# brian-kelley/CUDA-QR

Measured on AMD Instinct MI355X. Metric: fp64 GFLOP/s (% of roofline) + ||A-QR||_F/||A||_F, m x n QR at 1/2/4/8 GPUs, higher is better.
Workload: dtype f64; 1 GPU; C3: 16384x16384 square fp64 QR on 1 MI355X, nb=256; m=16384, n=16384, m_per_gpu=16384, nb=256, ib=32, input_buffers=31, input=uniform[0,1) counter-hash generator, seed 12+i, resident in HBM, collective=none

## Files before the change

### cuda-qr_amd/__init__.py

```python
import ctypes as C
import os

import numpy as np

HERE = os.path.dirname(os.path.abspath(__file__))
_which = os.environ.get("CUDA_QR_AMD_LIB", "")
LAB = _which == "lab" or _which.endswith(".so")
LAB_LIB_PATH = os.path.join(HERE, "libmi355xqr_lab.so")
LIB_PATH = (os.path.join(HERE, _which) if _which.endswith(".so") else LAB_LIB_PATH) if LAB else os.path.join(HERE, "libmi355xqr.so")
HEADER = os.path.join(os.path.dirname(HERE), "include", "mi355x_qr.h")

if not os.path.exists(LIB_PATH):
    raise ImportError(
        f"{LIB_PATH} is missing: build it with `make -C {HERE} all lab` (or python -c 'import __graft_entry__ as g; "
        "g.build()').  The HIP extension is mandatory; there is no CPU fallback.")

try:
    import torch
except Exception:
    pass

lib = C.CDLL(LIB_PATH)

QR_PROF_CLASSES = 4
# ... 39 lines not shown
_sig("qr_strerror", C.c_char_p, C.c_int)
_sig("qr_set_block_size", C.c_int, C.c_int, C.c_int)
_sig("qr_get_block_size", None, C.POINTER(C.c_int), C.POINTER(C.c_int))
_sig("qr_default_block_size", C.c_int, C.c_int, C.c_int, C.POINTER(C.c_int), C.POINTER(C.c_int))
_sig("qr_thin", C.c_int, _dp, C.c_int, C.c_int, _dp, _dp, C.c_int, C.c_int)
_fp = C.POINTER(C.c_float)
_sig("mmqr_f32_status", C.c_int, _fp, C.POINTER(_fp), C.c_int, C.c_int)
_sig("explicitQR_f32_status", C.c_int, _fp, _fp, _fp, _fp, C.c_int, C.c_int)
_sig("qr_thin_mgpu", C.c_int, _dp, C.c_int, C.c_int, _dp, _dp, C.c_int, C.c_int)
_sig("qr_release_cached_plans", C.c_int)
_sig("qr_tsqr_unique_id", C.c_int, _vp)
_sig("qr_tsqr_plan_create", C.c_int, C.POINTER(_vp), _vp, C.c_int, C.c_int, C.c_int, C.c_int, C.c_int)
_sig("qr_tsqr_plan_create_comm", C.c_int, C.POINTER(_vp), _vp, C.c_int, C.c_int, C.c_int, C.c_int, C.c_int)
_sig("qr_tsqr_plan_destroy", C.c_int, _vp)
_sig("qr_tsqr_factor_dev", C.c_int, _vp, _vp, C.c_int, _vp)
_sig("qr_tsqr_formq_dev", C.c_int, _vp, _vp, C.c_int, _vp, C.c_int)
_sig("qr_tsqr_local_dev", C.c_int, _vp, _vp, C.c_int)
_sig("qr_tsqr_exchange_buffers", C.c_int, _vp, C.POINTER(_vp), C.POINTER(_vp))
_sig("qr_tsqr_stacked_dev", C.c_int, _vp, _vp)
_sig("qr_tsqr_is_pipelined", C.c_int, _vp)
_sig("qr_tsqr_set_schedule", C.c_int, _vp, C.c_int)
_sig("qr_tsqr_gather_stats", C.c_int, _vp, C.POINTER(C.c_double))
_sig("qr_tsqr_factor_virtual_dev", C.c_int, C.POINTER(_vp), C.c_int, C.POINTER(_vp), C.c_int, C.POINTER(_vp))
_sig("qr_tsqr_factor_selfgather_dev", C.c_int, _vp, _vp, C.c_int, _vp)
_sig("qr_tsqr_sync", C.c_int, _vp)
_sig("qr_tsqr_stream", _vp, _vp)
_sig("qr_tsqr_comm_ranks", C.c_int, _vp, C.POINTER(C.c_int))
_sig("qr_tsqr_local_plan", _vp, _vp)
_sig("qr_tsqr_stacked_plan", _vp, _vp)
_sig("qr_plan_create", C.c_int, C.POINTER(_vp), C.c_int, C.c_int, C.c_int, C.c_int)
_sig("qr_plan_destroy", C.c_int, _vp)
_sig("qr_geqrf_dev", C.c_int, _vp, _vp, C.c_int, C.c_int, C.c_int, _vp)
_sig("qr_applyq_dev", C.c_int, _vp, _vp, C.c_int, C.c_int, C.c_int, _vp, _vp, C.c_int, C.c_int, C.c_int)
_sig("qr_build_t_dev", C.c_int, _vp, _vp, C.c_int, C.c_int, C.c_int, _vp, _vp, C.c_int)
_sig("qr_ormqr_dev", C.c_int, _vp, C.c_char, _vp, C.c_int, C.c_int, C.c_int, _vp, _vp, C.c_int, _vp, C.c_int, C.c_int)
_sig("qr_solve_r_dev", C.c_int, _vp, _vp, C.c_int, C.c_int, _vp, C.c_int, C.c_int)
_sig("qr_gels_dev", C.c_int, _vp, _vp, C.c_int, C.c_int, C.c_int, _vp, _vp, C.c_int, C.c_int)
_sig("qr_lstsq", C.c_int, _dp, C.c_int, C.c_int, _dp, C.c_int, _dp, _dp)
_sig("qr_extract_r_dev", C.c_int, _vp, _vp, C.c_int, C.c_int, C.c_int, _vp, C.c_int, C.c_int)
_sig("qr_gemm_dev", C.c_int, _vp, C.c_char, C.c_int, C.c_int, C.c_int, C.c_double, _vp, C.c_int, _vp, C.c_int,
     C.c_double, _vp, C.c_int)
_sig("qr_fill_uniform_dev", C.c_int, _vp, _vp, C.c_int, C.c_longlong, C.c_int, C.c_longlong, C.c_longlong,
     C.c_ulonglong)
_sig("qr_uniform_at", C.c_double, C.c_ulonglong, C.c_ulonglong)
_sig("qr_diffnorm_dev", C.c_int, _vp, _vp, C.c_int, _vp, C.c_int, C.c_longlong, C.c_int, C.c_longlong,
     C.c_longlong, C.c_ulonglong, C.c_int, _dp)
_sig("qr_device_malloc", C.c_int, C.POINTER(_vp), C.c_size_t)
_sig("qr_device_free", C.c_int, _vp)
_sig("qr_copy_to_device", C.c_int, _vp, _vp, C.c_size_t)
_sig("qr_copy_to_host", C.c_int, _vp, _vp, C.c_size_t)
_sig("qr_plan_sync", C.c_int, _vp)
_sig("qr_plan_stream", _vp, _vp)
_sig("qr_plan_set_guard_mode", C.c_int, _vp, C.c_int)
_sig("qr_plan_route_stats", C.c_int, _vp, C.POINTER(C.c_longlong))
_sig("qr_plan_retry_stats", C.c_int, _vp, C.POINTER(C.c_longlong))
_sig("qr_plan_info", C.c_int, _vp, C.POINTER(C.c_int), C.POINTER(C.c_int), C.POINTER(C.c_int))
_sig("qr_plan_update_cus", C.c_int, _vp)
_sig("qr_plan_set_profile", C.c_int, _vp, C.c_int)
_sig("qr_plan_pause_profile", C.c_int, _vp, C.c_int)
_sig("qr_plan_get_profile", C.c_int, _vp, C.POINTER(Profile))
_sig("qr_plan_get_profile_records", C.c_int, _vp, C.c_int, C.POINTER(C.c_int), _dp, _dp)
_sig("qr_device_info", C.c_int, C.c_char_p, C.c_int, C.POINTER(C.c_int), C.POINTER(C.c_int), C.POINTER(C.c_size_t))
_sig("qr_probe_mfma_f64_tflops", C.c_int, _dp)
_sig("qr_probe_copy_gbps", C.c_int, _dp)
_sig("qrd_gemm_nn", C.c_int, _vp, C.c_int, C.c_int, C.c_int, C.c_double, _vp, C.c_int, _vp, C.c_int, C.c_double,
     _vp, C.c_int)
_sig("qrd_gemm_tn", C.c_int, _vp, C.c_int, C.c_int, C.c_int, C.c_double, _vp, C.c_int, _vp, C.c_int, C.c_double,
     _vp, C.c_int, _vp, C.c_size_t, _vp, C.c_int)
_sig("qrd_gemm_tn_update", C.c_int, _vp, C.c_int, C.c_int, C.c_int, C.c_double, _vp, C.c_int, _vp, C.c_int, C.c_double,
     _vp, C.c_int, _vp, C.c_size_t)
_sig("qrd_gemm_tn_update_wide", C.c_int, _vp, C.c_int, C.c_int, C.c_int, C.c_double, _vp, C.c_int, _vp, C.c_int, C.c_double,
     _vp, C.c_int, _vp, C.c_size_t)
_sig("qrd_gemm_tn_dual", C.c_int, _vp, C.c_int, C.c_int, C.c_int, _vp, C.c_int, _vp, C.c_int, _vp, C.c_int, _vp, C.c_int, _vp, C.c_int, _vp, C.c_int,
     _vp, C.c_size_t)
_sig("qrd_trsm_gt", C.c_int, _vp, C.c_int, C.c_int, _vp, C.c_int, _vp, C.c_int, _vp, C.c_int, _vp, C.c_int)
_sig("qrd_larft", C.c_int, _vp, C.c_int, C.c_int, _vp, C.c_int, _vp, _vp, C.c_int, _vp, C.c_int, _vp, C.c_int)
_sig("qrd_panel_ws_size", C.c_size_t, C.c_int)
_sig("qrd_panel_tsqr", C.c_int, _vp, _vp, C.c_int, C.c_int, C.c_int, _vp, _vp, C.c_int, _vp, C.c_int, _vp, C.c_int)
_sig("qrd_panel_cholqr", C.c_int, _vp, _vp, C.c_int, C.c_int, C.c_int, _vp, _vp, C.c_int, _vp, C.c_int, _vp, C.c_int, _vp, _vp, C.c_size_t, C.c_int)
_sig("qrd_leaf_update_gram", C.c_int, _vp, C.c_int, C.c_int, _vp, C.c_int, _vp, _vp, C.c_int, _vp, C.c_size_t, C.c_int, C.POINTER(C.c_int))
_sig("qrd_gemm_nt", C.c_int, _vp, C.c_int, C.c_int, C.c_int, C.c_int, _vp, C.c_int, _vp, C.c_int, _vp, C.c_int, C.c_int, _vp)
if hasattr(lib, "qrd_gemm_nt4_ok"):
    _sig("qrd_gemm_nt4_ok", C.c_int, C.c_int, C.c_int, C.c_int, _vp, C.c_int, _vp, C.c_int, _vp, C.c_int)
_sig("qrd_copy_block", C.c_int, _vp, _vp, C.c_int, _vp, C.c_int, C.c_int, C.c_int)
_sig("qrd_init", C.c_int)
_sig("qrd_device_sync", C.c_int)


def strerror(rc):
    return lib.qr_strerror(rc).decode()


def check(rc, what=""):
    if rc != 0:
        raise QRError(f"{what or 'mi355xqr'} failed: {strerror(rc)} ({rc})", rc)


def exported_symbols():
    import re
    txt = open(HEADER).read()
    txt = re.sub(r"/\*.*?\*/", "", txt, flags=re.S)
    names = re.findall(r"^\s*(?:const\s+)?(?:int|void|double|char\*|void\*|const char\*|qr_plan\*)\s*\*?\s*(\w+)\s*\(", txt, flags=re.M)
    return sorted(set(names))


def _f(a):
    return np.asfortranarray(a, dtype=np.float64)


def _p(a):
    return a.ctypes.data_as(_dp)


def get_panel_dims(m, n):
    rp, cp = C.c_int(), C.c_int()
    lib.getPanelDims(m, n, C.byref(rp), C.byref(cp))
    return rp.value, cp.value


def get_block_size():
    nb, ib = C.c_int(), C.c_int()
    lib.qr_get_block_size(C.byref(nb), C.byref(ib))
    return nb.value, ib.value


def default_block_size(m, n):
    nb, ib = C.c_int(), C.c_int()
    check(lib.qr_default_block_size(m, n, C.byref(nb), C.byref(ib)), "qr_default_block_size")
    return nb.value, ib.value


def tau_len(m, n):
    rp, cp = get_panel_dims(m, n)
    return rp * cp * default_block_size(m, n)[0]


def set_block_size(nb, ib):
    check(lib.qr_set_block_size(nb, ib), "qr_set_block_size")


_libc = C.CDLL(None)
_libc.free.argtypes = [C.c_void_p]


def mmqr(A):
    F = np.array(A, dtype=np.float64, order="F", copy=True)
    m, n = F.shape
    tptr = _dp()
    check(lib.mmqr_status(_p(F), C.byref(tptr), m, n), "mmqr")
    tau = np.ctypeslib.as_array(tptr, shape=(tau_len(m, n),)).copy()
    _libc.free(C.cast(tptr, C.c_void_p))
    return F, tau


def explicit_qr(F, tau):
    F = _f(F)
    m, n = F.shape
    tau = np.ascontiguousarray(tau, dtype=np.float64)
    if tau.size < n:
        raise QRError(f"explicit_qr: tau has {tau.size} entries, the factorisation of {n} columns has {n}")
    Q = np.empty((m, m), order="F")
    R = np.empty((m, n), order="F")
    check(lib.explicitQR_status(_p(F), _p(tau), _p(Q), _p(R), m, n), "explicitQR")
    return Q, R


# ... 348 lines not shown
```

### cuda-qr_amd/csrc/qr_common.h

```cpp
#ifndef QR_COMMON_H
#define QR_COMMON_H
#include <hip/hip_runtime.h>

typedef double v4d __attribute__((ext_vector_type(4)));
typedef double v2d __attribute__((ext_vector_type(2)));

#define LEAFW 32

#ifdef QR_LAB
#include <stdlib.h>
#define QRD_LAB_ENV_INT(name, dflt) ([] { const char* e_ = getenv(name); return e_ ? atoi(e_) : (dflt); }())
#else
#define QRD_LAB_ENV_INT(name, dflt) (dflt)
#endif

__device__ __forceinline__ double dpp_f64(double v, int which)
{
    int lo = __double2loint(v), hi = __double2hiint(v);
    switch (which) {
    case 0: lo = __builtin_amdgcn_update_dpp(lo, lo, 0x140, 0xF, 0xF, false); hi = __builtin_amdgcn_update_dpp(hi, hi, 0x140, 0xF, 0xF, false); break;
    case 1: lo = __builtin_amdgcn_update_dpp(lo, lo, 0x141, 0xF, 0xF, false); hi = __builtin_amdgcn_update_dpp(hi, hi, 0x141, 0xF, 0xF, false); break;
    case 2: lo = __builtin_amdgcn_update_dpp(lo, lo, 0x4E, 0xF, 0xF, false); hi = __builtin_amdgcn_update_dpp(hi, hi, 0x4E, 0xF, 0xF, false); break;
    default: lo = __builtin_amdgcn_update_dpp(lo, lo, 0xB1, 0xF, 0xF, false); hi = __builtin_amdgcn_update_dpp(hi, hi, 0xB1, 0xF, 0xF, false); break;
    }
    return __hiloint2double(hi, lo);
}

template <bool SWAP32>
__device__ __forceinline__ double swap_add(double a, double b)
{
    const unsigned alo = (unsigned) __double2loint(a), ahi = (unsigned) __double2hiint(a);
    const unsigned blo = (unsigned) __double2loint(b), bhi = (unsigned) __double2hiint(b);
    if (SWAP32) {
        auto rl = __builtin_amdgcn_permlane32_swap(alo, blo, false, false);
        auto rh = __builtin_amdgcn_permlane32_swap(ahi, bhi, false, false);
        return __hiloint2double((int) rh[0], (int) rl[0]) + __hiloint2double((int) rh[1], (int) rl[1]);
    } else {
        auto rl = __builtin_amdgcn_permlane16_swap(alo, blo, false, false);
        auto rh = __builtin_amdgcn_permlane16_swap(ahi, bhi, false, false);
        return __hiloint2double((int) rh[0], (int) rl[0]) + __hiloint2double((int) rh[1], (int) rl[1]);
    }
}

__device__ __forceinline__ double wave_reduce32(const double (&a)[LEAFW], int lane)
{
    double b16[16], b8[8], b4[4], b2[2];
#pragma unroll
    for (int q = 0; q < 16; ++q) b16[q] = swap_add<true>(a[q], a[q + 16]);
#pragma unroll
    for (int q = 0; q < 8; ++q) b8[q] = swap_add<false>(b16[q], b16[q + 8]);
    {
        const bool up = (lane & 8) != 0;
#pragma unroll
        for (int q = 0; q < 4; ++q) {
            const double send = up ? b8[q] : b8[q + 4], keep = up ? b8[q + 4] : b8[q];
            b4[q] = keep + dpp_f64(send, 0);
        }
    }
    {
        const bool up = (lane & 4) != 0;
#pragma unroll
        for (int q = 0; q < 2; ++q) {
            const double send = up ? b4[q] : b4[q + 2], keep = up ? b4[q + 2] : b4[q];
            b2[q] = keep + dpp_f64(send, 1);
        }
    }
    const bool up = (lane & 2) != 0;
    double v = (up ? b2[1] : b2[0]) + dpp_f64(up ? b2[0] : b2[1], 2);
    v += dpp_f64(v, 3);
    return v;
}
__device__ __forceinline__ void tile_of_block(int bid, int gx, int gy, int gm, int& tx, int& ty)
{
    const int nwg = gx * gy;
    int id = bid;
    if (gm > 0) {
        const int q = nwg >> 3, r = nwg & 7, xcd = bid & 7, loc = bid >> 3;
        id = (xcd < r ? xcd * (q + 1) : r * (q + 1) + (xcd - r) * q) + loc;
        const int per = gm * gy, g = id / per, in = id - g * per;
        const int rows = min(gm, gx - g * gm);
        tx = g * gm + in % rows;
        ty = in / rows;
    } else {
        tx = id % gx;
        ty = id / gx;
    }
}

#endif
```

### cuda-qr_amd/csrc/qr_device.h

```cpp
#ifndef QR_DEVICE_H
#define QR_DEVICE_H
#include <stddef.h>
#ifdef __cplusplus
extern "C" {
#endif

int qrd_init(void);
int qrd_gemm_nn(void* stream, int M, int N, int K, double alpha, const double* A, int lda, const double* B,
                int ldb, double beta, double* C, int ldc);
int qrd_gemm_tn(void* stream, int M, int N, int K, double alpha, const double* A, int lda, const double* B,
                int ldb, double beta, double* C, int ldc, double* slabs, size_t slab_cap, const double* Tm,
                int ldt);
int qrd_gemm_nn_update(void* stream, int M, int N, int K, double alpha, const double* A, int lda, const double* B,
                       int ldb, double beta, double* C, int ldc);
int qrd_gemm_nn_update2(void* stream, int M, int N, int K, double alpha, const double* A, int lda, const double* B,
                        int ldb, double beta, double* C, int ldc);
int qrd_gemm_tn_dual(void* stream, int N1, int N2, int K, const double* A, int lda, const double* B1, int ldb1, const double* B2,
                     int ldb2, const double* Tm, int ldt, double* W, int ldw, double* G2, int ldg, double* slabs, size_t slab_cap);
int qrd_gemm_tn_update(void* stream, int M, int N, int K, double alpha, const double* A, int lda, const double* B,
                       int ldb, double beta, double* C, int ldc, double* slabs, size_t slab_cap);
int qrd_gemm_tn_update_wide(void* stream, int M, int N, int K, double alpha, const double* A, int lda, const double* B,
                            int ldb, double beta, double* C, int ldc, double* slabs, size_t slab_cap);
int qrd_gemm2_init(void);
int qrd_gemm_nt_ok(int M, int N, int K, const double* A, int lda, const double* Bt, int ldbt, const double* C, int ldc);
int qrd_gemm_nt4_ok(int M, int N, int K, const double* A, int lda, const double* Bt, int ldbt, const double* C, int ldc);
int qrd_gemm_nt(void* stream, int M, int N, int K, int sign, const double* A, int lda, const double* Bt, int ldbt,
                double* C, int ldc, int gm, unsigned long long* stamps);
size_t qrd_panel_ws_size(int m);
int qrd_panel_tsqr_init(void);
int qrd_panel_tsqr(void* stream, double* P, int ld, int mk, int w, double* tau, double* T, int ldt, double* Vw, int ldv,
                   double* ws, int m_cap);
int qrd_slab_reduce(void* stream, int M, int N, int nslab, const double* slabs, int lds, size_t stride, double* out, int ldo);
#define QRD_CHOLQR_WS (10 * 32 * 32 + 16)
int qrd_panel_cholqr(void* stream, double* P, int ld, int mk, int w, double* tau, double* T, int ldt, double* Vw, int ldv,
                     double* ws, int m_cap, double* cws, double* slabs, size_t slab_cap, int gram_nslab);
int qrd_panel_cholqr_ep(void* stream, double* P, int ld, int mk, int w, double* tau, double* T, int ldt, double* Vw, int ldv,
                        double* ws, int m_cap, double* cws, double* slabs, size_t slab_cap, int gram_nslab,
                        int N1, const double* B1, int ldb1, int N2, const double* B2, int ldb2, double* W, int ldw, double* G2, int ldg,
                        double* ep_slabs, size_t ep_slab_cap, int* did);
int qrd_leaf_fused_init(void);
int qrd_leaf_update_gram(void* stream, int mk, int N, const double* V, int ldv, const double* W, double* C, int ldc, double* gslabs,
                         size_t gslab_cap, int gy, int* nslab);
int qrd_gemm_nn_batch(void* stream, int M, int N, int K, double alpha, const double* A, int lda, size_t sA,
                      const double* B, int ldb, size_t sB, double beta, double* C, int ldc, size_t sC, int batch);
int qrd_larft(void* stream, int nbp, int ib, const double* G, int ldg, const double* tau, double* T, int ldt,
              double* Tt, int build_diag, double* X, int ldx);
int qrd_zero_block(void* stream, double* A, int ld, int rows, int cols);
int qrd_trsm_gt(void* stream, int kw, int nc, const double* G, int ldg, const double* T, int ldt, const double* Y, int ldy, double* W, int ldw);
int qrd_transpose(void* stream, int rows, int cols, const double* S, int lds, double* D, int ldd);
int qrd_extract_v(void* stream, const double* P, int ld, int mk, int w, double* V, int ldv);
int qrd_extract_r(void* stream, const double* A, int lda, int m, int n, double* R, int ldr, int rrows);
int qrd_extract_r_block(void* stream, const double* A, int lda, int k, int w, double* R, int ldr, int rrows);
int qrd_set_identity(void* stream, double* C, int ld, int rows, int cols, int row_off);
int qrd_copy_block(void* stream, const double* S, int lds, double* D, int ldd, int rows, int cols);
int qrd_copy_blocks(void* stream, const double* S, int lds, size_t sstride, double* D, int ldd, size_t dstride, int rows, int cols, int batch);
int qrd_fill_uniform(void* stream, double* A, int ld, long long rows, int cols, long long row_off,
                     long long total_rows, unsigned long long seed);
double qrd_hash_uniform_host(unsigned long long seed, unsigned long long idx);
int qrd_diff_norm(void* stream, const double* X, int ldx, const double* Y, int ldy, long long rows, int cols,
                  long long row_off, long long total_rows, unsigned long long seed, int sub_identity, double* out);

size_t qrd_panel_cqr_ws_doubles(void);
int qrd_panel_cqr_init(void);
int qrd_panel_cqr_ok(int mk, int w);
int qrd_panel_cqr(void* stream, double* A, int lda, int mk, int w, double* tau, double* T, int ldt, double* Vw, int ldv, double* ws, int* status);
int qrd_panel_cqr_q(void* stream, double* A, int lda, int mk, int w, double* tau, double* T, int ldt, double* Vw, int ldv, double* ws, int* status,
                    double* Qb, int ldq, unsigned* hflag, unsigned seq);
int qrd_panel_cqr_p(void* stream, double* A, int lda, int mk, int w, double* tau, double* T, int ldt, double* Vw, int ldv, double* ws, int* status,
                    double* Qb, int ldq, unsigned* hflag, unsigned seq, int park);
int qrd_panel_cqr_retry(void* stream, double* A, int lda, int mk, int w, double* tau, double* T, int ldt, double* Vw, int ldv, double* ws, int* status,
                    double* Qb, int ldq, unsigned* hflag, unsigned seq, int park);
int qrd_panel_cqr_restore_r(void* stream, double* A, int lda, int w, const double* ws, const int* status);
int qrd_panel_cqr_r_block(void* stream, const double* ws, int w, double* D, int ldd);
double* qrd_panel_cqr_g1(double* ws);
double* qrd_panel_cqr_g2(double* ws);
int qrd_panel_cqr_stage1(void* stream, const double* A, int lda, int mk, int w, double* Vw, int ldv, double* ws, int* status);
int qrd_panel_cqr_stage2(void* stream, double* A, int lda, int mk, int w, double* tau, double* T, int ldt, double* Vw, int ldv, double* ws,
                         int* status);
size_t qrd_panel_fused_ws_doubles(void);
int qrd_panel_fused_init(void);
int qrd_panel_fused_merges_t(int wh, int with_gram);
int qrd_panel_fused_ok(void* stream, const double* A, int lda, int mk, int wh, const double* Vw, int ldv);
int qrd_panel_fused(void* stream, double* A, int lda, int mk, int wh, double* tau, double* T, int ldt, double* Vw, int ldv,
                    double* G, int ldg, double* ws, unsigned* epoch, int* status);
int qrd_panel_fused_rows(void* stream, double* A, int lda, int mk, int wh, double* tau, double* T, int ldt, double* Vw, int ldv,
                    double* G, int ldg, double* ws, unsigned* epoch, int* status, int want_rows);

size_t qrd_legacy_ws_size(int m, int PR, int PC);
int qrd_legacy_shape_ok(int m, int n, int PR, int PC);
int qrd_legacy_panel(void* stream, double* A, int m, int n, int PR, int PC, int rowPanels, int pc, int pcCount, double* tau, double* wy);
int qrd_legacy_formq(void* stream, const double* A, const double* tau, int m, int n, int PR, int PC, int rowPanels, double* Q);

#define QRD_E_NORCCL (-120)
#define QRD_E_RCCL   (-130)
#define QRD_UNIQUE_ID_BYTES 128
int qrd_comm_init_all(void** comms, int n, const int* devs);
int qrd_comm_unique_id(void* id);
int qrd_comm_init_rank(void** comm, int nranks, const void* id, int rank);
int qrd_comm_count(void* comm, int* n);
const char* qrd_rccl_error_string(int r);
int qrd_comm_destroy(void* comm);
int qrd_allgather_f64(void* comm, void* stream, const double* send, double* recv, size_t count);

void qrd_range_push(const char* name);
void qrd_range_pop(void);

int qrd_malloc(void** p, size_t bytes);
int qrd_free(void* p);
int qrd_memset(void* stream, void* p, int v, size_t bytes);
int qrd_h2d(void* stream, void* d, const void* h, size_t bytes);
// ... 49 lines not shown
```

### cuda-qr_amd/csrc/qr_gemm_nt.hip

```cpp
#include <hip/hip_runtime.h>
#include <stdint.h>
#include <stdlib.h>
#include "qr_device.h"
#include "qr_common.h"

#define NT_BM 128
#define NT_BN 128
#define NT_BK 16
#define NT_STAGE (2 * NT_BK * 128)

#define GLOBAL_PTR(p) ((const __attribute__((address_space(1))) void*) (p))
#define LDS_PTR(p) ((__attribute__((address_space(3))) void*) (p))


template <bool NEG, int STAMP, int IL = 0, int CEIL = 0>
__global__ __launch_bounds__(512, 4) void gemm_nt_kernel(int M, int N, int K, const double* __restrict__ A, int lda,
                                                         const double* __restrict__ Bt, int ldbt,
                                                         double* __restrict__ C, int ldc, int gx, int gy, int gm,
                                                         unsigned long long* __restrict__ stamps)
{
    extern __shared__ __attribute__((aligned(16))) double smem[];
    const int tid = threadIdx.x, lane = tid & 63, wave = tid >> 6;
    const int wi = wave & 1, wj = wave >> 1;
    const int l15 = lane & 15, l4 = lane >> 4;
// ... 90 lines not shown
            for (int j = 0; j < 8; ++j) {
                mm(0, j);
                if (j == 0) rd(1, st, 1, 0); else if (j == 2) rd(1, st, 1, 1); else if (j == 4) rd(1, st, 1, 2);
                else if (j == 1) ld(kt + 1, sn, 0); else if (j == 3) ld(kt + 1, sn, 1); else if (j == 5) ld(kt + 1, sn, 2);
                else if (j == 7) ld(kt + 1, sn, 3);
                NT_SB;
            }
#pragma unroll
            for (int j = 0; j < 8; ++j) {
                mm(1, j);
                if (j == 0) rd(0, st, 2, 0); else if (j == 2) rd(0, st, 2, 1); else if (j == 4) rd(0, st, 2, 2);
                NT_SB;
            }
#pragma unroll
            for (int j = 0; j < 8; ++j) {
                mm(0, j);
                if (j == 0) rd(1, st, 3, 0); else if (j == 2) rd(1, st, 3, 1); else if (j == 4) rd(1, st, 3, 2);
                NT_SB;
            }
#pragma unroll
            for (int j = 0; j < 4; ++j) { mm(1, j); NT_SB; }
            __syncthreads();
            NT_SB;
#pragma unroll
            for (int j = 4; j < 8; ++j) {
                mm(1, j);
                if (j < 7) rd(0, stn, 0, j - 4);
                NT_SB;
            }
        }
        {
            const double* st = smem + ((nk - 1) & 1) * NT_STAGE + l4 * 128;
#pragma unroll
            for (int j = 0; j < 8; ++j) { mm(0, j); if (j == 0) rd(1, st, 1, 0); else if (j == 2) rd(1, st, 1, 1); else if (j == 4) rd(1, st, 1, 2); NT_SB; }
#pragma unroll
            for (int j = 0; j < 8; ++j) { mm(1, j); if (j == 0) rd(0, st, 2, 0); else if (j == 2) rd(0, st, 2, 1); else if (j == 4) rd(0, st, 2, 2); NT_SB; }
#pragma unroll
            for (int j = 0; j < 8; ++j) { mm(0, j); if (j == 0) rd(1, st, 3, 0); else if (j == 2) rd(1, st, 3, 1); else if (j == 4) rd(1, st, 3, 2); NT_SB; }
#pragma unroll
            for (int j = 0; j < 8; ++j) mm(1, j);
        }
#undef NT_SB
    } else
    for (int kt = 0; kt < nk; ++kt) {
        if (kt + 1 < nk) issue(kt + 1, (kt + 1) & 1);
        const double* st = smem + (kt & 1) * NT_STAGE + l4 * 128;
        NT_READ(0, 0);
        NT_READ(1, 1);
        __builtin_amdgcn_sched_barrier(0);
        NT_MMA(0);
        __builtin_amdgcn_sched_barrier(0);
        NT_READ(0, 2);
        __builtin_amdgcn_sched_barrier(0);
        NT_MMA(1);
        __builtin_amdgcn_sched_barrier(0);
        NT_READ(1, 3);
        __builtin_amdgcn_sched_barrier(0);
        NT_MMA(0);
        NT_MMA(1);
        __syncthreads();
    }
#undef NT_READ
#undef NT_MMA
    if (STAMP) t2 = __builtin_amdgcn_s_memtime();

#pragma unroll
    for (int a = 0; a < 2; ++a)
#pragma unroll
        for (int c = 0; c < 2; ++c)
#pragma unroll
            for (int r = 0; r < 4; ++r) {
                if (CEIL) { if (acc[a][2 * c][r] == 0.12345678) *reinterpret_cast<v2d*>(cp[a] + 32 * c + 8 * r) = (v2d){acc[a][2 * c][r], acc[a][2 * c + 1][r]}; }
                else *reinterpret_cast<v2d*>(cp[a] + 32 * c + 8 * r) = (v2d){acc[a][2 * c][r], acc[a][2 * c + 1][r]};
            }
    if (STAMP && tid == 0) {
        const unsigned long long t3 = __builtin_amdgcn_s_memtime();
        unsigned long long* s = stamps + 6 * (size_t) blockIdx.x;
        const unsigned hw = __builtin_amdgcn_s_getreg((4) | (0 << 6) | ((32 - 1) << 11));
        const unsigned xcc = __builtin_amdgcn_s_getreg((20) | (0 << 6) | ((4 - 1) << 11));
        s[0] = t0; s[1] = t1; s[2] = t2; s[3] = t3; s[4] = (unsigned long long) hw | ((unsigned long long) (xcc & 0xf) << 32); s[5] = blockIdx.x;
    }
}

template <bool NEG, int CEIL, int BK4, int NS, bool RAG = false>
__global__ __launch_bounds__(256, (BK4 == 8 ? 4 : 3)) void gemm_nt4_kernel(int M, int N, int K, const double* __restrict__ A, int lda,
                                                          const double* __restrict__ Bt, int ldbt,
                                                          double* __restrict__ C, int ldc, int gx, int gy, int gm)
{
    constexpr int STAGE = BK4 * 128 + BK4 * 64;
    constexpr int NLD = 3 * BK4 / 8;
    extern __shared__ __attribute__((aligned(16))) double smem[];
    const int tid = threadIdx.x, lane = tid & 63, wave = __builtin_amdgcn_readfirstlane(tid >> 6);
    const int wi = wave & 1, wj = wave >> 1;
    const int l15 = lane & 15, l4 = lane >> 4;
    int tx, ty;
    tile_of_block(blockIdx.x, gx, gy, gm, tx, ty);
    const int i0 = tx * 128, j0 = ty * 64;
    const double* ga = A + (size_t) wave * lda + i0 + 2 * lane;
    const double* gb = Bt + (size_t) (2 * wave + (lane >> 5)) * ldbt + j0 + 2 * (lane & 31);
    auto issue = [&](int kt, int stage) {
        if (CEIL == 2) return;
        const double* pa = ga + (size_t) kt * BK4 * lda;
        const double* pb = gb + (size_t) kt * BK4 * ldbt;
        double* sa = smem + stage * STAGE;
#pragma unroll
        for (int q = 0; q < BK4 / 4; ++q)
            __builtin_amdgcn_global_load_lds(GLOBAL_PTR(pa + (size_t) (4 * q) * lda), LDS_PTR(sa + (wave + 4 * q) * 128), 16, 0, 0);
#pragma unroll
        for (int q = 0; q < BK4 / 8; ++q)
            __builtin_amdgcn_global_load_lds(GLOBAL_PTR(pb + (size_t) (8 * q) * ldbt), LDS_PTR(sa + BK4 * 128 + (wave + 4 * q) * 128), 16, 0, 0);
    };
    const int nk = K / BK4;
    issue(0, 0);
    if (NS == 3 && nk > 1) issue(1, 1);
    __builtin_amdgcn_sched_barrier(0);
    v4d acc[2][4];
    double* cp[2];
    const int rlim = RAG ? M - (i0 + 64 * wi + 2 * l4) : 0;
#pragma unroll
    for (int a = 0; a < 2; ++a) {
        cp[a] = C + (size_t) (j0 + 32 * wj + 2 * l15 + a) * ldc + i0 + 64 * wi + 2 * l4;
#pragma unroll
        for (int c = 0; c < 2; ++c)
#pragma unroll
            for (int r = 0; r < 4; ++r) {
                const v2d v = (CEIL || (RAG && 32 * c + 8 * r >= rlim)) ? (v2d){1.0, 2.0} : *reinterpret_cast<const v2d*>(cp[a] + 32 * c + 8 * r);
                acc[a][2 * c][r] = v[0];
                acc[a][2 * c + 1][r] = v[1];
            }
    }
    __syncthreads();
    const int aoff = 64 * wi + 2 * l15 + l4 * 128, boff = BK4 * 128 + 32 * wj + 2 * l15 + l4 * 64;
    constexpr int NKS = BK4 / 4;
    v2d fa[NKS][2], fb[NKS];
    if constexpr (BK4 == 8 && NS == 3) {
        auto rd = [&](int set, const double* st_, int ks, int which) {
            if (which == 0) fa[set][0] = *reinterpret_cast<const v2d*>(st_ + ks * 4 * 128 + aoff);
            else if (which == 1) fb[set] = *reinterpret_cast<const v2d*>(st_ + ks * 4 * 64 + boff);
            else fa[set][1] = *reinterpret_cast<const v2d*>(st_ + ks * 4 * 128 + aoff + 32);
        };
        auto mm = [&](int set, int j) {
            const int a = j >> 2, b = j & 3;
            acc[a][b] = __builtin_amdgcn_mfma_f64_16x16x4f64(fa[set][b >> 1][b & 1], fb[set][a], acc[a][b], 0, 0, NEG ? 1 : 0);
        };
        auto ld = [&](int kt_, int q) {
            if (CEIL == 2) return;
            const double* pa = ga + (size_t) kt_ * BK4 * lda;
            const double* pb = gb + (size_t) kt_ * BK4 * ldbt;
            double* sa = smem + (kt_ % 3) * STAGE;
            if (q == 0) __builtin_amdgcn_global_load_lds(GLOBAL_PTR(pa), LDS_PTR(sa + wave * 128), 16, 0, 0);
            else if (q == 1) __builtin_amdgcn_global_load_lds(GLOBAL_PTR(pa + (size_t) 4 * lda), LDS_PTR(sa + (wave + 4) * 128), 16, 0, 0);
            else __builtin_amdgcn_global_load_lds(GLOBAL_PTR(pb), LDS_PTR(sa + BK4 * 128 + wave * 128), 16, 0, 0);
        };
#define N4_SB __builtin_amdgcn_sched_barrier(0)
        rd(0, smem, 0, 0); rd(0, smem, 0, 1); rd(0, smem, 0, 2);
        N4_SB;
        for (int kt = 0; kt + 1 < nk; ++kt) {
            const double* st = smem + (kt % 3) * STAGE;
            const double* stn = smem + ((kt + 1) % 3) * STAGE;
            const bool more = kt + 2 < nk;
#pragma unroll
            for (int j = 0; j < 8; ++j) {
                mm(0, j);
                if (j == 0) rd(1, st, 1, 0); else if (j == 2) rd(1, st, 1, 1); else if (j == 4) rd(1, st, 1, 2);
                else if (more && j == 1) ld(kt + 2, 0); else if (more && j == 3) ld(kt + 2, 1); else if (more && j == 5) ld(kt + 2, 2);
                N4_SB;
            }
#pragma unroll
            for (int j = 0; j < 4; ++j) { mm(1, j); N4_SB; }
            if (more) asm volatile("s_waitcnt vmcnt(3)" ::: "memory");
            else asm volatile("s_waitcnt vmcnt(0)" ::: "memory");
            __builtin_amdgcn_fence(__ATOMIC_RELEASE, "workgroup", "local");
            __builtin_amdgcn_s_barrier();
            __builtin_amdgcn_fence(__ATOMIC_ACQUIRE, "workgroup", "local");
            N4_SB;
#pragma unroll
            for (int j = 4; j < 8; ++j) {
                mm(1, j);
                if (j < 7) rd(0, stn, 0, j - 4);
                N4_SB;
            }
        }
        {
            const double* st = smem + ((nk - 1) % 3) * STAGE;
#pragma unroll
            for (int j = 0; j < 8; ++j) { mm(0, j); if (j == 0) rd(1, st, 1, 0); else if (j == 2) rd(1, st, 1, 1); else if (j == 4) rd(1, st, 1, 2); N4_SB; }
#pragma unroll
            for (int j = 0; j < 8; ++j) mm(1, j);
        }
#undef N4_SB
    } else
    for (int kt = 0; kt < nk; ++kt) {
        const int stage = kt % NS;
        if (kt + NS - 1 < nk) issue(kt + NS - 1, (kt + NS - 1) % NS);
        const double* st = smem + stage * STAGE;
#pragma unroll
        for (int ks = 0; ks < NKS; ++ks) {
            fa[ks][0] = *reinterpret_cast<const v2d*>(st + ks * 4 * 128 + aoff);
            fa[ks][1] = *reinterpret_cast<const v2d*>(st + ks * 4 * 128 + aoff + 32);
            fb[ks] = *reinterpret_cast<const v2d*>(st + ks * 4 * 64 + boff);
        }
        __builtin_amdgcn_sched_barrier(0);
#pragma unroll
        for (int ks = 0; ks < NKS; ++ks)
#pragma unroll
            for (int a = 0; a < 2; ++a) {
                acc[a][0] = __builtin_amdgcn_mfma_f64_16x16x4f64(fa[ks][0][0], fb[ks][a], acc[a][0], 0, 0, NEG ? 1 : 0);
                acc[a][1] = __builtin_amdgcn_mfma_f64_16x16x4f64(fa[ks][0][1], fb[ks][a], acc[a][1], 0, 0, NEG ? 1 : 0);
                acc[a][2] = __builtin_amdgcn_mfma_f64_16x16x4f64(fa[ks][1][0], fb[ks][a], acc[a][2], 0, 0, NEG ? 1 : 0);
                acc[a][3] = __builtin_amdgcn_mfma_f64_16x16x4f64(fa[ks][1][1], fb[ks][a], acc[a][3], 0, 0, NEG ? 1 : 0);
            }
        if (NS == 3 && kt + 2 < nk) asm volatile("s_waitcnt vmcnt(%0)" ::"n"(NLD) : "memory");
        else asm volatile("s_waitcnt vmcnt(0)" ::: "memory");
        __builtin_amdgcn_fence(__ATOMIC_RELEASE, "workgroup", "local");
        __builtin_amdgcn_s_barrier();
        __builtin_amdgcn_fence(__ATOMIC_ACQUIRE, "workgroup", "local");
    }
#pragma unroll
    for (int a = 0; a < 2; ++a)
#pragma unroll
        for (int c = 0; c < 2; ++c)
#pragma unroll
            for (int r = 0; r < 4; ++r) {
                if (RAG && 32 * c + 8 * r >= rlim) continue;
                if (CEIL) { if (acc[a][2 * c][r] == 0.12345678) *reinterpret_cast<v2d*>(cp[a] + 32 * c + 8 * r) = (v2d){acc[a][2 * c][r], acc[a][2 * c + 1][r]}; }
                else *reinterpret_cast<v2d*>(cp[a] + 32 * c + 8 * r) = (v2d){acc[a][2 * c][r], acc[a][2 * c + 1][r]};
            }
}

static int nt4(void)
{
    static const int v = QRD_LAB_ENV_INT("MI355XQR_NT4", 1);
    return v;
}

#ifdef QR_LAB
static int nt_ceil(void)
{
    static const int v = QRD_LAB_ENV_INT("MI355XQR_NT_CEIL", 0);
    return v;
}
#endif


static int nt_gm(void)
{
    static const int v = 8;
    return v;
}

static int nt_il(void)
{
    static const int v = QRD_LAB_ENV_INT("MI355XQR_NT_IL", 1);
    return v;
}

static inline bool al16(const void* p, int ld) { return (((uintptr_t) p) & 15) == 0 && (ld & 1) == 0; }

extern "C" {

int qrd_gemm2_init(void)
{
    int rc = 0;
    rc |= (int) hipFuncSetAttribute(reinterpret_cast<const void*>(gemm_nt_kernel<true, 0>), hipFuncAttributeMaxDynamicSharedMemorySize, 100 * 1024);
    rc |= (int) hipFuncSetAttribute(reinterpret_cast<const void*>(gemm_nt_kernel<false, 0>), hipFuncAttributeMaxDynamicSharedMemorySize, 2 * NT_STAGE * 8);
    rc |= (int) hipFuncSetAttribute(reinterpret_cast<const void*>(gemm_nt_kernel<true, 1>), hipFuncAttributeMaxDynamicSharedMemorySize, 2 * NT_STAGE * 8);
    rc |= (int) hipFuncSetAttribute(reinterpret_cast<const void*>(gemm_nt_kernel<true, 0, 1>), hipFuncAttributeMaxDynamicSharedMemorySize, 100 * 1024);
    rc |= (int) hipFuncSetAttribute(reinterpret_cast<const void*>(gemm_nt4_kernel<true, 0, 8, 3>), hipFuncAttributeMaxDynamicSharedMemorySize, 3 * 8 * 192 * 8);
    rc |= (int) hipFuncSetAttribute(reinterpret_cast<const void*>(gemm_nt4_kernel<true, 0, 8, 3, true>), hipFuncAttributeMaxDynamicSharedMemorySize, 3 * 8 * 192 * 8);
#ifdef QR_LAB
    rc |= (int) hipFuncSetAttribute(reinterpret_cast<const void*>(gemm_nt_kernel<true, 0, 1, 1>), hipFuncAttributeMaxDynamicSharedMemorySize, 100 * 1024);
    rc |= (int) hipFuncSetAttribute(reinterpret_cast<const void*>(gemm_nt_kernel<true, 0, 1, 2>), hipFuncAttributeMaxDynamicSharedMemorySize, 100 * 1024);
    rc |= (int) hipFuncSetAttribute(reinterpret_cast<const void*>(gemm_nt4_kernel<true, 1, 8, 3>), hipFuncAttributeMaxDynamicSharedMemorySize, 3 * 8 * 192 * 8);
    rc |= (int) hipFuncSetAttribute(reinterpret_cast<const void*>(gemm_nt4_kernel<true, 2, 8, 3>), hipFuncAttributeMaxDynamicSharedMemorySize, 3 * 8 * 192 * 8);
    rc |= (int) hipFuncSetAttribute(reinterpret_cast<const void*>(gemm_nt4_kernel<true, 0, 16, 2>), hipFuncAttributeMaxDynamicSharedMemorySize, 2 * 16 * 192 * 8);
    rc |= (int) hipFuncSetAttribute(reinterpret_cast<const void*>(gemm_nt4_kernel<true, 1, 16, 2>), hipFuncAttributeMaxDynamicSharedMemorySize, 2 * 16 * 192 * 8);
    rc |= (int) hipFuncSetAttribute(reinterpret_cast<const void*>(gemm_nt4_kernel<true, 2, 16, 2>), hipFuncAttributeMaxDynamicSharedMemorySize, 2 * 16 * 192 * 8);
#endif
    return rc;
}

int qrd_gemm_nt_ok(int M, int N, int K, const double* A, int lda, const double* Bt, int ldbt, const double* C, int ldc)
{
    return M >= 128 && N >= 128 && M % 128 == 0 && N % 128 == 0 && K >= 16 && K % 16 == 0 && al16(A, lda) && al16(Bt, ldbt) && al16(C, ldc);
}

int qrd_gemm_nt4_ok(int M, int N, int K, const double* A, int lda, const double* Bt, int ldbt, const double* C, int ldc)
{
    if (nt4() != 1) return qrd_gemm_nt_ok(M, N, K, A, lda, Bt, ldbt, C, ldc);
    if (M < 128 || N < 64 || N % 64 || K < 32 || K % 16 || !al16(A, lda) || !al16(Bt, ldbt) || !al16(C, ldc)) return 0;
    if (M % 128 == 0) return 1;
    return M % 2 == 0 && (M + 127) / 128 * 128 <= lda;
}

int qrd_gemm_nt(void* stream, int M, int N, int K, int sign, const double* A, int lda, const double* Bt, int ldbt,
                double* C, int ldc, int gm, unsigned long long* stamps)
{
    if (!stamps && sign < 0 && nt4() == 1 && !qrd_gemm_nt_ok(M, N, K, A, lda, Bt, ldbt, C, ldc) && qrd_gemm_nt4_ok(M, N, K, A, lda, Bt, ldbt, C, ldc)) {
        const int gx4 = (M + 127) / 128, gy4 = N / 64;
        if (gm < 0) gm = nt_gm();
        if (M % 128)
            hipLaunchKernelGGL((gemm_nt4_kernel<true, 0, 8, 3, true>), dim3(gx4 * gy4), dim3(256), 3 * (8 * 192) * sizeof(double), (hipStream_t) stream,
                               M, N, K, A, lda, Bt, ldbt, C, ldc, gx4, gy4, gm);
        else
            hipLaunchKernelGGL((gemm_nt4_kernel<true, 0, 8, 3>), dim3(gx4 * gy4), dim3(256), 3 * (8 * 192) * sizeof(double), (hipStream_t) stream,
                               M, N, K, A, lda, Bt, ldbt, C, ldc, gx4, gy4, gm);
        return (int) hipGetLastError();
    }
    if (!qrd_gemm_nt_ok(M, N, K, A, lda, Bt, ldbt, C, ldc)) return -7;
    const int gx = M / 128, gy = N / 128;
    if (gm < 0) gm = nt_gm();
    static const int solo = 0;
    const size_t shm = solo ? (size_t) 100 * 1024 : 2 * NT_STAGE * sizeof(double);
    hipStream_t s = (hipStream_t) stream;
    if (!stamps && sign < 0 && nt4() && K >= 32) {
        const int gy4 = N / 64;
        const dim3 g(gx * gy4), b(256);
#define NT4_LAUNCH(CE, BK, NS) hipLaunchKernelGGL((gemm_nt4_kernel<true, CE, BK, NS>), g, b, NS * (BK * 192) * sizeof(double), s, M, N, K, A, lda, Bt, ldbt, C, ldc, gx, gy4, gm)
#ifdef QR_LAB
        if (nt4() == 2) { if (nt_ceil() == 1) NT4_LAUNCH(1, 16, 2); else if (nt_ceil() == 2) NT4_LAUNCH(2, 16, 2); else NT4_LAUNCH(0, 16, 2); }
        else { if (nt_ceil() == 1) NT4_LAUNCH(1, 8, 3); else if (nt_ceil() == 2) NT4_LAUNCH(2, 8, 3); else NT4_LAUNCH(0, 8, 3); }
#else
        NT4_LAUNCH(0, 8, 3);
#endif
#undef NT4_LAUNCH
        return (int) hipGetLastError();
    }
#ifdef QR_LAB
    if (!stamps && sign < 0 && nt_ceil() == 1) {
        hipLaunchKernelGGL((gemm_nt_kernel<true, 0, 1, 1>), dim3(gx * gy), dim3(512), shm, s, M, N, K, A, lda, Bt, ldbt, C, ldc, gx, gy, gm, stamps);
        return (int) hipGetLastError();
    }
    if (!stamps && sign < 0 && nt_ceil() == 2) {
        hipLaunchKernelGGL((gemm_nt_kernel<true, 0, 1, 2>), dim3(gx * gy), dim3(512), shm, s, M, N, K, A, lda, Bt, ldbt, C, ldc, gx, gy, gm, stamps);
        return (int) hipGetLastError();
    }
#endif
    if (stamps)
        hipLaunchKernelGGL((gemm_nt_kernel<true, 1>), dim3(gx * gy), dim3(512), shm, s, M, N, K, A, lda, Bt, ldbt, C, ldc, gx, gy, gm, stamps);
    else if (sign < 0 && nt_il())
        hipLaunchKernelGGL((gemm_nt_kernel<true, 0, 1>), dim3(gx * gy), dim3(512), shm, s, M, N, K, A, lda, Bt, ldbt, C, ldc, gx, gy, gm, stamps);
    else if (sign < 0)
        hipLaunchKernelGGL((gemm_nt_kernel<true, 0>), dim3(gx * gy), dim3(512), shm, s, M, N, K, A, lda, Bt, ldbt, C, ldc, gx, gy, gm, stamps);
    else
        hipLaunchKernelGGL((gemm_nt_kernel<false, 0>), dim3(gx * gy), dim3(512), shm, s, M, N, K, A, lda, Bt, ldbt, C, ldc, gx, gy, gm, stamps);
    return (int) hipGetLastError();
}

}
```

Before: 49890 GFLOP/s.

## Add persistent NT GEMM with dedicated C-streaming wave and leaner barriers

Adds gemm_ntc_kernel, a persistent 320-thread kernel. Four waves run MFMA over a strip of tiles per workgroup and accumulate into an LDS C tile, while a fifth wave streams the previous tile's result out to global memory and preloads the next tile's C into LDS. The goal is to hide C read/write traffic behind compute and cut launch and tail overhead. This path is selected only when MI355XQR_NT4=3, which only the lab build can set. Separately, the existing nt4 kernel now uses a bare s_waitcnt lgkmcnt(0) plus s_barrier in place of the workgroup release/acquire fences by default. That trims fence overhead but relies on the hand-written waitcnt being enough for correctness.

```diff
diff --git a/cuda-qr_amd/__init__.py b/cuda-qr_amd/__init__.py
--- a/cuda-qr_amd/__init__.py
+++ b/cuda-qr_amd/__init__.py
@@ -145,6 +145,8 @@
 _sig("qrd_gemm_nt", C.c_int, _vp, C.c_int, C.c_int, C.c_int, C.c_int, _vp, C.c_int, _vp, C.c_int, _vp, C.c_int, C.c_int, _vp)
 if hasattr(lib, "qrd_gemm_nt4_ok"):
     _sig("qrd_gemm_nt4_ok", C.c_int, C.c_int, C.c_int, C.c_int, _vp, C.c_int, _vp, C.c_int, _vp, C.c_int)
+if hasattr(lib, "qrd_gemm_ntc"):
+    _sig("qrd_gemm_ntc", C.c_int, _vp, C.c_int, C.c_int, C.c_int, _vp, C.c_int, _vp, C.c_int, _vp, C.c_int, C.c_int, C.c_int)
 _sig("qrd_copy_block", C.c_int, _vp, _vp, C.c_int, _vp, C.c_int, C.c_int, C.c_int)
 _sig("qrd_init", C.c_int)
 _sig("qrd_device_sync", C.c_int)
diff --git a/cuda-qr_amd/csrc/qr_common.h b/cuda-qr_amd/csrc/qr_common.h
--- a/cuda-qr_amd/csrc/qr_common.h
+++ b/cuda-qr_amd/csrc/qr_common.h
@@ -70,13 +70,9 @@
     v += dpp_f64(v, 3);
     return v;
 }
-__device__ __forceinline__ void tile_of_block(int bid, int gx, int gy, int gm, int& tx, int& ty)
+__device__ __forceinline__ void tile_of_id(int id, int gx, int gy, int gm, int& tx, int& ty)
 {
-    const int nwg = gx * gy;
-    int id = bid;
     if (gm > 0) {
-        const int q = nwg >> 3, r = nwg & 7, xcd = bid & 7, loc = bid >> 3;
-        id = (xcd < r ? xcd * (q + 1) : r * (q + 1) + (xcd - r) * q) + loc;
         const int per = gm * gy, g = id / per, in = id - g * per;
         const int rows = min(gm, gx - g * gm);
         tx = g * gm + in % rows;
@@ -87,4 +83,15 @@
     }
 }
 
+__device__ __forceinline__ void tile_of_block(int bid, int gx, int gy, int gm, int& tx, int& ty)
+{
+    const int nwg = gx * gy;
+    int id = bid;
+    if (gm > 0) {
+        const int q = nwg >> 3, r = nwg & 7, xcd = bid & 7, loc = bid >> 3;
+        id = (xcd < r ? xcd * (q + 1) : r * (q + 1) + (xcd - r) * q) + loc;
+    }
+    tile_of_id(id, gx, gy, gm, tx, ty);
+}
+
 #endif
diff --git a/cuda-qr_amd/csrc/qr_device.h b/cuda-qr_amd/csrc/qr_device.h
--- a/cuda-qr_amd/csrc/qr_device.h
+++ b/cuda-qr_amd/csrc/qr_device.h
@@ -26,6 +26,7 @@
 int qrd_gemm_nt4_ok(int M, int N, int K, const double* A, int lda, const double* Bt, int ldbt, const double* C, int ldc);
 int qrd_gemm_nt(void* stream, int M, int N, int K, int sign, const double* A, int lda, const double* Bt, int ldbt,
                 double* C, int ldc, int gm, unsigned long long* stamps);
+int qrd_gemm_ntc(void* stream, int M, int N, int K, const double* A, int lda, const double* Bt, int ldbt, double* C, int ldc, int gm, int strip);
 size_t qrd_panel_ws_size(int m);
 int qrd_panel_tsqr_init(void);
 int qrd_panel_tsqr(void* stream, double* P, int ld, int mk, int w, double* tau, double* T, int ldt, double* Vw, int ldv,
diff --git a/cuda-qr_amd/csrc/qr_gemm_nt.hip b/cuda-qr_amd/csrc/qr_gemm_nt.hip
--- a/cuda-qr_amd/csrc/qr_gemm_nt.hip
+++ b/cuda-qr_amd/csrc/qr_gemm_nt.hip
@@ -196,7 +196,7 @@
     }
 }
 
-template <bool NEG, int CEIL, int BK4, int NS, bool RAG = false>
+template <bool NEG, int CEIL, int BK4, int NS, bool RAG = false, bool BARE = true>
 __global__ __launch_bounds__(256, (BK4 == 8 ? 4 : 3)) void gemm_nt4_kernel(int M, int N, int K, const double* __restrict__ A, int lda,
                                                           const double* __restrict__ Bt, int ldbt,
                                                           double* __restrict__ C, int ldc, int gx, int gy, int gm)
@@ -284,9 +284,15 @@
             for (int j = 0; j < 4; ++j) { mm(1, j); N4_SB; }
             if (more) asm volatile("s_waitcnt vmcnt(3)" ::: "memory");
             else asm volatile("s_waitcnt vmcnt(0)" ::: "memory");
-            __builtin_amdgcn_fence(__ATOMIC_RELEASE, "workgroup", "local");
-            __builtin_amdgcn_s_barrier();
-            __builtin_amdgcn_fence(__ATOMIC_ACQUIRE, "workgroup", "local");
+            if constexpr (BARE) {
+                asm volatile("s_waitcnt lgkmcnt(0)" ::: "memory");
+                __builtin_amdgcn_s_barrier();
+                asm volatile("" ::: "memory");
+            } else {
+                __builtin_amdgcn_fence(__ATOMIC_RELEASE, "workgroup", "local");
+                __builtin_amdgcn_s_barrier();
+                __builtin_amdgcn_fence(__ATOMIC_ACQUIRE, "workgroup", "local");
+            }
             N4_SB;
 #pragma unroll
             for (int j = 4; j < 8; ++j) {
@@ -342,9 +348,183 @@
             }
 }
 
+#define NTC_STG (3 * 8 * 192)
+#define NTC_BARRIER()                                             \
+    do {                                                          \
+        asm volatile("s_waitcnt lgkmcnt(0)" ::: "memory");        \
+        __builtin_amdgcn_s_barrier();                             \
+        asm volatile("" ::: "memory");                            \
+    } while (0)
+template <bool RAG>
+__global__ __launch_bounds__(320, 1) void gemm_ntc_kernel(int M, int N, int K, const double* __restrict__ A, int lda,
+                                                          const double* __restrict__ Bt, int ldbt,
+                                                          double* __restrict__ C, int ldc, int gx, int gy, int gm, int strip)
+{
+    constexpr int BK4 = 8, STAGE = BK4 * 192;
+    extern __shared__ __attribute__((aligned(16))) double smem[];
+    double* const stg = smem + NTC_STG;
+    const int tid = threadIdx.x, lane = tid & 63, wave = __builtin_amdgcn_readfirstlane(tid >> 6);
+    const int nwg = gx * gy, xq = nwg >> 3, xr = nwg & 7, xcd = blockIdx.x & 7, loc = blockIdx.x >> 3;
+    const int start = xcd < xr ? xcd * (xq + 1) : xr * (xq + 1) + (xcd - xr) * xq, cnt = xq + (xcd < xr);
+    const int first = (loc >> 5) * strip * 32 + (loc & 31);
+    if (first >= cnt) return;
+    const int nt = min(strip, (cnt - first + 31) >> 5);
+    const int nk = K / BK4;
+
+    if (wave == 4) {
+        int tx = 0, ty = 0, px = 0, py = 0;
+        auto cols4 = [&](int j, bool st, bool ld) {
+            v2d v[4];
+            int p[4];
+#pragma unroll
+            for (int q = 0; q < 4; ++q) {
+                p[q] = lane ^ (((j + q) >> 1) & 15);
+                if (st) v[q] = *reinterpret_cast<const v2d*>(stg + (j + q) * 128 + 2 * lane);
+            }
+            asm volatile("s_waitcnt lgkmcnt(0)" ::: "memory");
+#pragma unroll
+            for (int q = 0; q < 4; ++q) {
+                if (st && (!RAG || px * 128 + 2 * p[q] < M)) *reinterpret_cast<v2d*>(C + (size_t) (py * 64 + j + q) * ldc + px * 128 + 2 * p[q]) = v[q];
+                if (ld && (!RAG || tx * 128 + 2 * p[q] < M))
+                    __builtin_amdgcn_global_load_lds(GLOBAL_PTR(C + (size_t) (ty * 64 + j + q) * ldc + tx * 128 + 2 * p[q]), LDS_PTR(stg + (j + q) * 128), 16, 0, 0);
+            }
+        };
+        auto bar = [&]() {
+            NTC_BARRIER();
+        };
+        tile_of_id(start + first, gx, gy, gm, tx, ty);
+        for (int j = 0; j < 64; j += 4) cols4(j, false, true);
+        bar();
+        const int wk = max(1, 2 * (nk - 1) / 3), cpi = ((64 + wk - 1) / wk + 3) & ~3;
+        for (int t = 0; t < nt; ++t) {
+            if (t) { px = tx; py = ty; tile_of_id(start + first + 32 * t, gx, gy, gm, tx, ty); }
+            int j = 0;
+            for (int kt = 0; kt < nk; ++kt) {
+                if (kt == nk - 1) {
+                    if (t) for (; j < 64; j += 4) cols4(j, true, true);
+                    asm volatile("s_waitcnt vmcnt(0)" ::: "memory");
+                } else if (t) {
+                    const int je = min(64, j + cpi);
+                    for (; j < je; j += 4) cols4(j, true, true);
+                }
+                bar();
+            }
+            bar();
+        }
+        px = tx; py = ty;
+        for (int j = 0; j < 64; j += 4) cols4(j, true, false);
+        return;
+    }
+
+    const int wi = wave & 1, wj = wave >> 1;
+    const int l15 = lane & 15, l4 = lane >> 4;
+    const int ng = nt * nk;
+    int lt = 0, lk = 0, ls = 0;
+    const double *ga, *gb;
+    auto load_tile = [&]() {
+        int tx, ty;
+        tile_of_id(start + first + 32 * lt, gx, gy, gm, tx, ty);
+        ga = A + (size_t) wave * lda + tx * 128 + 2 * lane;
+        gb = Bt + (size_t) (2 * wave + (lane >> 5)) * ldbt + ty * 64 + 2 * (lane & 31);
+    };
+    auto ld = [&](int q) {
+        const double* pa = ga + (size_t) lk * BK4 * lda;
+        const double* pb = gb + (size_t) lk * BK4 * ldbt;
+        double* sa = smem + ls * STAGE;
+        if (q == 0) __builtin_amdgcn_global_load_lds(GLOBAL_PTR(pa), LDS_PTR(sa + wave * 128), 16, 0, 0);
+        else if (q == 1) __builtin_amdgcn_global_load_lds(GLOBAL_PTR(pa + (size_t) 4 * lda), LDS_PTR(sa + (wave + 4) * 128), 16, 0, 0);
+        else __builtin_amdgcn_global_load_lds(GLOBAL_PTR(pb), LDS_PTR(sa + BK4 * 128 + wave * 128), 16, 0, 0);
+    };
+    auto ld_next = [&]() {
+        ls = ls == 2 ? 0 : ls + 1;
+        if (++lk == nk) { lk = 0; ++lt; if (lt < nt) load_tile(); }
+    };
+    load_tile();
+    ld(0); ld(1); ld(2); ld_next();
+    if (ng > 1) { ld(0); ld(1); ld(2); ld_next(); }
+    v4d acc[2][4];
+#pragma unroll
+    for (int a = 0; a < 2; ++a)
+#pragma unroll
+        for (int b = 0; b < 4; ++b) acc[a][b] = (v4d){0.0, 0.0, 0.0, 0.0};
+    double* sl[4];
+#pragma unroll
+    for (int r = 0; r < 4; ++r) sl[r] = stg + (32 * wj + 2 * l15) * 128 + 2 * (32 * wi + ((4 * r + l4) ^ l15));
+    asm volatile("s_waitcnt vmcnt(0)" ::: "memory");
+    NTC_BARRIER();
+    const int aoff = 64 * wi + 2 * l15 + l4 * 128, boff = BK4 * 128 + 32 * wj + 2 * l15 + l4 * 64;
+    v2d fa[2][2], fb[2];
+    auto rd = [&](int set, const double* st_, int ks, int which) {
+        if (which == 0) fa[set][0] = *reinterpret_cast<const v2d*>(st_ + ks * 4 * 128 + aoff);
+        else if (which == 1) fb[set] = *reinterpret_cast<const v2d*>(st_ + ks * 4 * 64 + boff);
+        else fa[set][1] = *reinterpret_cast<const v2d*>(st_ + ks * 4 * 128 + aoff + 32);
+    };
+    auto mm = [&](int set, int j) {
+        const int a = j >> 2, b = j & 3;
+        acc[a][b] = __builtin_amdgcn_mfma_f64_16x16x4f64(fa[set][b >> 1][b & 1], fb[set][a], acc[a][b], 0, 0, 1);
+    };
+#define NC_SB __builtin_amdgcn_sched_barrier(0)
+    rd(0, smem, 0, 0); rd(0, smem, 0, 1); rd(0, smem, 0, 2);
+    NC_SB;
+    int cs = 0, kt = 0;
+    for (int g = 0; g < ng; ++g) {
+        const double* st = smem + cs * STAGE;
+        cs = cs == 2 ? 0 : cs + 1;
+        const double* stn = smem + cs * STAGE;
+        const bool more = g + 2 < ng;
+#pragma unroll
+        for (int j = 0; j < 8; ++j) {
+            mm(0, j);
+            if (j == 0) rd(1, st, 1, 0); else if (j == 2) rd(1, st, 1, 1); else if (j == 4) rd(1, st, 1, 2);
+            else if (more && j == 1) ld(0); else if (more && j == 3) ld(1); else if (more && j == 5) ld(2);
+            NC_SB;
+        }
+        if (more) ld_next();
+#pragma unroll
+        for (int j = 0; j < 4; ++j) { mm(1, j); NC_SB; }
+        if (more) asm volatile("s_waitcnt vmcnt(3)" ::: "memory");
+        else asm volatile("s_waitcnt vmcnt(0)" ::: "memory");
+        NTC_BARRIER();
+        NC_SB;
+#pragma unroll
+        for (int j = 4; j < 8; ++j) {
+            mm(1, j);
+            if (j < 7) rd(0, stn, 0, j - 4);
+            NC_SB;
+        }
+        if (++kt == nk) {
+            kt = 0;
+#pragma unroll
+            for (int a = 0; a < 2; ++a)
+#pragma unroll
+                for (int c = 0; c < 2; ++c)
+#pragma unroll
+                    for (int r = 0; r < 4; ++r) {
+                        v2d* p = reinterpret_cast<v2d*>(sl[r] + a * 128 + c * 32);
+                        v2d v = *p;
+                        v[0] += acc[a][2 * c][r];
+                        v[1] += acc[a][2 * c + 1][r];
+                        *p = v;
+                        acc[a][2 * c][r] = 0.0;
+                        acc[a][2 * c + 1][r] = 0.0;
+                    }
+            NTC_BARRIER();
+            NC_SB;
+        }
+    }
+#undef NC_SB
+#undef NTC_BARRIER
+}
+
 static int nt4(void)
 {
     static const int v = QRD_LAB_ENV_INT("MI355XQR_NT4", 1);
+    return v;
+}
+
+static int ntc_strip(void)
+{
+    static const int v = QRD_LAB_ENV_INT("MI355XQR_NTC_STRIP", 8);
     return v;
 }
 
@@ -382,9 +562,12 @@
     rc |= (int) hipFuncSetAttribute(reinterpret_cast<const void*>(gemm_nt_kernel<true, 0, 1>), hipFuncAttributeMaxDynamicSharedMemorySize, 100 * 1024);
     rc |= (int) hipFuncSetAttribute(reinterpret_cast<const void*>(gemm_nt4_kernel<true, 0, 8, 3>), hipFuncAttributeMaxDynamicSharedMemorySize, 3 * 8 * 192 * 8);
     rc |= (int) hipFuncSetAttribute(reinterpret_cast<const void*>(gemm_nt4_kernel<true, 0, 8, 3, true>), hipFuncAttributeMaxDynamicSharedMemorySize, 3 * 8 * 192 * 8);
+    rc |= (int) hipFuncSetAttribute(reinterpret_cast<const void*>(gemm_ntc_kernel<false>), hipFuncAttributeMaxDynamicSharedMemorySize, (NTC_STG + 128 * 64) * 8);
+    rc |= (int) hipFuncSetAttribute(reinterpret_cast<const void*>(gemm_ntc_kernel<true>), hipFuncAttributeMaxDynamicSharedMemorySize, (NTC_STG + 128 * 64) * 8);
 #ifdef QR_LAB
     rc |= (int) hipFuncSetAttribute(reinterpret_cast<const void*>(gemm_nt_kernel<true, 0, 1, 1>), hipFuncAttributeMaxDynamicSharedMemorySize, 100 * 1024);
     rc |= (int) hipFuncSetAttribute(reinterpret_cast<const void*>(gemm_nt_kernel<true, 0, 1, 2>), hipFuncAttributeMaxDynamicSharedMemorySize, 100 * 1024);
+    rc |= (int) hipFuncSetAttribute(reinterpret_cast<const void*>(gemm_nt4_kernel<true, 0, 8, 3, false, false>), hipFuncAttributeMaxDynamicSharedMemorySize, 3 * 8 * 192 * 8);
     rc |= (int) hipFuncSetAttribute(reinterpret_cast<const void*>(gemm_nt4_kernel<true, 1, 8, 3>), hipFuncAttributeMaxDynamicSharedMemorySize, 3 * 8 * 192 * 8);
     rc |= (int) hipFuncSetAttribute(reinterpret_cast<const void*>(gemm_nt4_kernel<true, 2, 8, 3>), hipFuncAttributeMaxDynamicSharedMemorySize, 3 * 8 * 192 * 8);
     rc |= (int) hipFuncSetAttribute(reinterpret_cast<const void*>(gemm_nt4_kernel<true, 0, 16, 2>), hipFuncAttributeMaxDynamicSharedMemorySize, 2 * 16 * 192 * 8);
@@ -401,16 +584,37 @@
 
 int qrd_gemm_nt4_ok(int M, int N, int K, const double* A, int lda, const double* Bt, int ldbt, const double* C, int ldc)
 {
-    if (nt4() != 1) return qrd_gemm_nt_ok(M, N, K, A, lda, Bt, ldbt, C, ldc);
+    if (nt4() != 1 && nt4() != 3) return qrd_gemm_nt_ok(M, N, K, A, lda, Bt, ldbt, C, ldc);
     if (M < 128 || N < 64 || N % 64 || K < 32 || K % 16 || !al16(A, lda) || !al16(Bt, ldbt) || !al16(C, ldc)) return 0;
     if (M % 128 == 0) return 1;
     return M % 2 == 0 && (M + 127) / 128 * 128 <= lda;
 }
 
+int qrd_gemm_ntc(void* stream, int M, int N, int K, const double* A, int lda, const double* Bt, int ldbt, double* C, int ldc, int gm, int strip)
+{
+    if (M < 128 || N < 64 || N % 64 || K < 32 || K % 16 || !al16(A, lda) || !al16(Bt, ldbt) || !al16(C, ldc)) return -7;
+    if (M % 128 && (M % 2 || (M + 127) / 128 * 128 > lda)) return -7;
+    const int gx = (M + 127) / 128, gy = N / 64;
+    if (gm < 0) gm = nt_gm();
+    if (strip <= 0) strip = ntc_strip();
+    const int per_xcd = (gx * gy + 7) / 8, blocks = (per_xcd + 32 * strip - 1) / (32 * strip);
+    const dim3 g(8 * 32 * blocks), b(320);
+    const size_t shm = (NTC_STG + 128 * 64) * sizeof(double);
+    if (M % 128)
+        hipLaunchKernelGGL((gemm_ntc_kernel<true>), g, b, shm, (hipStream_t) stream, M, N, K, A, lda, Bt, ldbt, C, ldc, gx, gy, gm, strip);
+    else
+        hipLaunchKernelGGL((gemm_ntc_kernel<false>), g, b, shm, (hipStream_t) stream, M, N, K, A, lda, Bt, ldbt, C, ldc, gx, gy, gm, strip);
+    return (int) hipGetLastError();
+}
+
 int qrd_gemm_nt(void* stream, int M, int N, int K, int sign, const double* A, int lda, const double* Bt, int ldbt,
                 double* C, int ldc, int gm, unsigned long long* stamps)
 {
-    if (!stamps && sign < 0 && nt4() == 1 && !qrd_gemm_nt_ok(M, N, K, A, lda, Bt, ldbt, C, ldc) && qrd_gemm_nt4_ok(M, N, K, A, lda, Bt, ldbt, C, ldc)) {
+    if (!stamps && sign < 0 && nt4() == 3 && K >= 128) {
+        const int rc = qrd_gemm_ntc(stream, M, N, K, A, lda, Bt, ldbt, C, ldc, gm, 0);
+        if (rc != -7) return rc;
+    }
+    if (!stamps && sign < 0 && (nt4() == 1 || nt4() == 3) && !qrd_gemm_nt_ok(M, N, K, A, lda, Bt, ldbt, C, ldc) && qrd_gemm_nt4_ok(M, N, K, A, lda, Bt, ldbt, C, ldc)) {
         const int gx4 = (M + 127) / 128, gy4 = N / 64;
         if (gm < 0) gm = nt_gm();
         if (M % 128)
@@ -433,6 +637,7 @@
 #define NT4_LAUNCH(CE, BK, NS) hipLaunchKernelGGL((gemm_nt4_kernel<true, CE, BK, NS>), g, b, NS * (BK * 192) * sizeof(double), s, M, N, K, A, lda, Bt, ldbt, C, ldc, gx, gy4, gm)
 #ifdef QR_LAB
         if (nt4() == 2) { if (nt_ceil() == 1) NT4_LAUNCH(1, 16, 2); else if (nt_ceil() == 2) NT4_LAUNCH(2, 16, 2); else NT4_LAUNCH(0, 16, 2); }
+        else if (nt4() == 4) hipLaunchKernelGGL((gemm_nt4_kernel<true, 0, 8, 3, false, false>), g, b, 3 * (8 * 192) * sizeof(double), s, M, N, K, A, lda, Bt, ldbt, C, ldc, gx, gy4, gm);
         else { if (nt_ceil() == 1) NT4_LAUNCH(1, 8, 3); else if (nt_ceil() == 2) NT4_LAUNCH(2, 8, 3); else NT4_LAUNCH(0, 8, 3); }
 #else
         NT4_LAUNCH(0, 8, 3);
```

Result: no change. 50220 GFLOP/s, median of 6 (+0.7%).
